# CloudEngineHub/dexrobot_isaac

Measured on AMD Instinct MI355X. Metric: env-steps/sec BlindGrasping num_envs=4096 per MI355X (random actions), higher is better.
Workload: dtype f32

## Files before the change

dexrobot_isaac_amd/csrc/dexsim_device.h:

```cpp
#pragma once
#include <hip/hip_runtime.h>

#include "../../include/dexsim.h"

#define DEXSIM_FIELDS(X)                                                                                    \
                                \
  X(float, q, 26) X(float, qd, 26) X(float, targets, 26)                                                    \
  X(float, box_pos, 3) X(float, box_quat, 4) X(float, box_lin, 3) X(float, box_ang, 3)                      \
  X(float, box_mass, 1) X(float, box_mu, 1)                                                                 \
                                                \
  X(float, site_pose, 77) X(float, hand_vel, 6) X(float, cforce, 51) X(float, cf5, 15)                      \
                                                    \
  X(float, jframe, 156) X(float, ufree, 32) X(float, fac_finv, 60)                                          \
  X(float, fac_g, 120) X(int, ncontact, 1) X(float, cgeom, DEXSIM_KMAX * 8) X(int, ccode, DEXSIM_KMAX)      \
  X(float, crow, DEXSIM_KMAX * 3 * 28) X(float, crowq, DEXSIM_KMAX * 3 * 28 + 4) X(float, clam, DEXSIM_KMAX * 3) X(float, chdr, DEXSIM_KMAX * 8) X(float, cstage, 6 * NP_STAGE * 9)                                         \
   \
  X(float, wlam, DEXSIM_NWKEY * 4) X(int, wgen, 1) X(int, csplit, 1)                                         \
        \
  X(float, active_prev_targets, 18) X(float, active_rule_targets, 18) X(float, prev_actions, 18)            \
  X(float, actions, 18) X(float, prev_dof_pos, 26)                                                          \
  X(float, contact_duration_steps, 5) X(float, prev_contact_binary, 5) X(int, episode_step, 1)              \
  X(int, success_duration_steps, 1) X(int, success_conditions_met, 1) X(int, current_stage, 1)              \
  X(int, just2, 1) X(int, just3, 1) X(float, time_in_stage, 1) X(float, stage_contact_duration, 1)          \
  X(float, initial_box_pos, 3)                                                                              \
  X(float, prev_finger_dof_vel, 20) X(float, prev_hand_vel, 3) X(float, prev_hand_ang_vel, 3)               \
  X(int, prev_contacts, 5)                                                                                  \
  X(int, episode_success, 1) X(int, episode_failure, 1) X(int, success_reason, DEXSIM_NUM_SUCC)             \
  X(int, failure_reason, DEXSIM_NUM_FAIL) X(int, crit_success, DEXSIM_NUM_SUCC)                             \
  X(int, crit_failure, DEXSIM_NUM_FAIL) X(int, term_success, 1) X(int, term_failure, 1)                     \
  X(int, term_timeout, 1)                                                                                   \
  X(float, obs_all, DEXSIM_OBS_ALL_DIM) X(float, rew_comp, DEXSIM_NUM_REWROWS) X(float, rew, 1)             \
  X(int, reset_flag, 1) X(int, reset_count, 1)

struct Arena {
#define X(type, name, rows) type* name;
  DEXSIM_FIELDS(X)
#undef X
};

#define FQ(field, quad) ((__attribute__((address_space(1))) f4*)(A.field) + ((size_t)(quad) * N + e))
#define JFRAME_FQ0 9
#define NP_STAGE 20
#define CSTAGE_CODE0 (6 * NP_STAGE * 8)

#define CROW_W 28

struct JC {
  float qoff[4], poff[3], axis[3], com[3], inertia[6];
  float mass, kp, kd, armature, lo, hi;
  float pad[7];
};
static_assert(sizeof(JC) == 128, "JC must be 128 bytes");

struct DevParams {
  DexSimConfig cfg;
  DexHandModel model;
  float h;
  float box_inv_I_k;
  float base_A[4][3], base_Oc[4][3], base_Q3z[4];
  unsigned obs_div_magic;
  int inertia_diag;
  float hand_reach;
  int obs_col_row[DEXSIM_OBS_ALL_DIM];
  JC jc[DEXSIM_NJ];
  Arena arena;
};

#define CNT_ANY_RESET 0
#define CNT_SUCC 1
#define CNT_FAIL 2
#define CNT_TERM_SUCCESS 8
#define CNT_TERM_FAILURE 9
#define CNT_TERM_TIMEOUT 10
#define CNT_NUM_RESETS 11
#define CNT_CONTACTS 16
#define CNT_HAND_CONTACTS 18
#define CNT_SPIN_TIMEOUT 20
#define CNT_PHYS_STEPS 13
#define CNT_CONSECUTIVE 14
#define CNT_RC_FIRST 15

typedef float f2 __attribute__((ext_vector_type(2)));
typedef float f4 __attribute__((ext_vector_type(4)));
__device__ __forceinline__ void st4_global(float* p, f4 v) { *(__attribute__((address_space(1))) f4*)p = v; }
__device__ __forceinline__ void st4_global(float* p, float a, float b, float c, float d) { f4 v; v.x = a; v.y = b; v.z = c; v.w = d; st4_global(p, v); }

struct V3 { float x, y, z; };
struct Q4 { float x, y, z, w; };
struct S6 { float xx, yy, zz, xy, xz, yz; };
struct M3 { float m[9]; };

#define DI __device__ __forceinline__

DI V3 v3(float x, float y, float z) { return {x, y, z}; }
DI V3 v3p(const float* p) { return {p[0], p[1], p[2]}; }
DI V3 operator+(V3 a, V3 b) { return {a.x + b.x, a.y + b.y, a.z + b.z}; }
DI V3 operator-(V3 a, V3 b) { return {a.x - b.x, a.y - b.y, a.z - b.z}; }
DI V3 operator*(float s, V3 a) { return {s * a.x, s * a.y, s * a.z}; }
DI V3& operator+=(V3& a, V3 b) { a.x += b.x; a.y += b.y; a.z += b.z; return a; }
DI V3& operator-=(V3& a, V3 b) { a.x -= b.x; a.y -= b.y; a.z -= b.z; return a; }
DI float dot(V3 a, V3 b) { return a.x * b.x + a.y * b.y + a.z * b.z; }
DI V3 cross(V3 a, V3 b) { return {a.y * b.z - a.z * b.y, a.z * b.x - a.x * b.z, a.x * b.y - a.y * b.x}; }
DI float norm(V3 a) { return sqrtf(dot(a, a)); }
DI float clampf(float x, float lo, float hi) { return x < lo ? lo : (x > hi ? hi : x); }

DI Q4 q4p(const float* p) { return {p[0], p[1], p[2], p[3]}; }
DI Q4 qmul(Q4 a, Q4 b) {
  return {a.w * b.x + a.x * b.w + a.y * b.z - a.z * b.y, a.w * b.y - a.x * b.z + a.y * b.w + a.z * b.x,
          a.w * b.z + a.x * b.y - a.y * b.x + a.z * b.w, a.w * b.w - a.x * b.x - a.y * b.y - a.z * b.z};
}
DI Q4 qconj(Q4 a) { return {-a.x, -a.y, -a.z, a.w}; }
DI M3 q2mat(Q4 q) {
  M3 R;
  float x = q.x, y = q.y, z = q.z, w = q.w;
  R.m[0] = 1 - 2 * (y * y + z * z); R.m[1] = 2 * (x * y - z * w); R.m[2] = 2 * (x * z + y * w);
  R.m[3] = 2 * (x * y + z * w); R.m[4] = 1 - 2 * (x * x + z * z); R.m[5] = 2 * (y * z - x * w);
  R.m[6] = 2 * (x * z - y * w); R.m[7] = 2 * (y * z + x * w); R.m[8] = 1 - 2 * (x * x + y * y);
  return R;
}
DI V3 mul(const M3& R, V3 v) {
  return {R.m[0] * v.x + R.m[1] * v.y + R.m[2] * v.z, R.m[3] * v.x + R.m[4] * v.y + R.m[5] * v.z,
          R.m[6] * v.x + R.m[7] * v.y + R.m[8] * v.z};
}
DI V3 mulT(const M3& R, V3 v) {
  return {R.m[0] * v.x + R.m[3] * v.y + R.m[6] * v.z, R.m[1] * v.x + R.m[4] * v.y + R.m[7] * v.z,
          R.m[2] * v.x + R.m[5] * v.y + R.m[8] * v.z};
}
DI V3 qrot_inv(Q4 q, V3 v) {
  V3 qv = {q.x, q.y, q.z};
  V3 c = cross(qv, v);
  float d = dot(qv, v), s = 2 * q.w * q.w - 1;
  return {v.x * s - 2 * q.w * c.x + 2 * qv.x * d, v.y * s - 2 * q.w * c.y + 2 * qv.y * d,
          v.z * s - 2 * q.w * c.z + 2 * qv.z * d};
}
DI V3 mul(S6 I, V3 v) {
  return {I.xx * v.x + I.xy * v.y + I.xz * v.z, I.xy * v.x + I.yy * v.y + I.yz * v.z,
          I.xz * v.x + I.yz * v.y + I.zz * v.z};
}
DI S6 operator+(S6 a, S6 b) { return {a.xx + b.xx, a.yy + b.yy, a.zz + b.zz, a.xy + b.xy, a.xz + b.xz, a.yz + b.yz}; }
DI S6 rotate_inertia(const M3& R, const float* s ) {
  float Il[9] = {s[0], s[3], s[4], s[3], s[1], s[5], s[4], s[5], s[2]};
  float T[9];
#pragma unroll
  for (int r = 0; r < 3; r++)
#pragma unroll
    for (int k = 0; k < 3; k++) T[3 * r + k] = R.m[3 * r] * Il[k] + R.m[3 * r + 1] * Il[3 + k] + R.m[3 * r + 2] * Il[6 + k];
  auto e = [&](int r, int k) { return T[3 * r] * R.m[3 * k] + T[3 * r + 1] * R.m[3 * k + 1] + T[3 * r + 2] * R.m[3 * k + 2]; };
  return {e(0, 0), e(1, 1), e(2, 2), e(0, 1), e(0, 2), e(1, 2)};
}
DI S6 rotate_inertia_diag(const M3& R, const float* s ) {
  const float a0 = s[0] * R.m[0], a3 = s[0] * R.m[3], a6 = s[0] * R.m[6];
  const float b1 = s[1] * R.m[1], b4 = s[1] * R.m[4], b7 = s[1] * R.m[7];
  const float c2 = s[2] * R.m[2], c5 = s[2] * R.m[5], c8 = s[2] * R.m[8];
  return {a0 * R.m[0] + b1 * R.m[1] + c2 * R.m[2], a3 * R.m[3] + b4 * R.m[4] + c5 * R.m[5], a6 * R.m[6] + b7 * R.m[7] + c8 * R.m[8],
          a0 * R.m[3] + b1 * R.m[4] + c2 * R.m[5], a0 * R.m[6] + b1 * R.m[7] + c2 * R.m[8], a3 * R.m[6] + b4 * R.m[7] + c5 * R.m[8]};
}
DI S6 pa(float m, V3 d) {
  float dd = dot(d, d);
  return {m * (dd - d.x * d.x), m * (dd - d.y * d.y), m * (dd - d.z * d.z), -m * d.x * d.y, -m * d.x * d.z, -m * d.y * d.z};
}

struct Comp { float m; V3 c; S6 I; };
DI void comp_add(Comp& a, const Comp& b) {
  float m = a.m + b.m;
  if (m <= 0.f) return;
  float inv = 1.f / m;
  V3 c = {(a.m * a.c.x + b.m * b.c.x) * inv, (a.m * a.c.y + b.m * b.c.y) * inv, (a.m * a.c.z + b.m * b.c.z) * inv};
  S6 I = a.I + b.I + pa(a.m * b.m * inv, a.c - b.c);
  a.m = m; a.c = c; a.I = I;
}

template <int n>
DI void spd_inverse(float* A) {
  float L[n * n];
#pragma unroll
  for (int i = 0; i < n; i++)
#pragma unroll
    for (int j = 0; j <= i; j++) {
      float s = A[i * n + j];
#pragma unroll
      for (int k = 0; k < j; k++) s -= L[i * n + k] * L[j * n + k];
      if (i == j) L[i * n + i] = sqrtf(fmaxf(s, 1e-20f));
      else L[i * n + j] = s / L[j * n + j];
    }
  float Li[n * n];
#pragma unroll
// ... 88 lines not shown
```

dexrobot_isaac_amd/csrc/dexsim_l2.hip.inc:

```

struct CouplingGroup { int n, dof[3]; float scale[3]; };
constexpr CouplingGroup kCoupling[18] = {
    {1, {0}, {1}}, {1, {1}, {1}}, {1, {2}, {1}}, {1, {3}, {1}}, {1, {4}, {1}}, {1, {5}, {1}},
    {1, {6}, {1}},
    {1, {7}, {1}},
    {2, {8, 9}, {1, 1}},
    {3, {10, 18, 22}, {1, 1, 2}},
    {1, {11}, {1}}, {2, {12, 13}, {1, 1}},
    {1, {15}, {1}}, {2, {16, 17}, {1, 1}},
    {1, {19}, {1}}, {2, {20, 21}, {1, 1}},
    {1, {23}, {1}}, {2, {24, 25}, {1, 1}},
};
constexpr int kHeldDof = 14;
constexpr int kActiveFingerDof[12] = {8, 7, 6, 10, 12, 11, 16, 15, 20, 19, 24, 23};

enum {
#define X(name, dim) O_##name, O_##name##_last = O_##name + (dim) - 1,
  DEXSIM_OBS_KEYS(X)
#undef X
  O_end
};
static_assert(O_end == DEXSIM_OBS_ALL_DIM, "DEXSIM_OBS_ALL_DIM is not the sum of the DEXSIM_OBS_KEYS dims");
static_assert(O_object_pos == DEXSIM_OBS_BASE_TASK_DIM, "DEXSIM_OBS_BASE_TASK_DIM is not the row of object_pos");

// ... 557 lines not shown
#pragma unroll 4
      for (int i = DEXSIM_OBS_BASE_TASK_DIM; i < DEXSIM_OBS_ALL_DIM; i++) OB(i) = 0.f;
    }
    post_logic_a(A, T, P, s_ob, in, mid, obs_only, N, NR);
  } else {
    if (wv == nw - 1)
      for (int i = lane; i < C.num_obs; i += 64) s_tab[i] = P->obs_col_row[i];
#pragma unroll 1
    for (int t = 0; t < POST_NTASK; t++)
      if (!((done_mask >> t) & 1) && (nw == 7 ? c_post_task_wave7[t] : c_post_task_wave[t] % nh) == wv - 1)
        post_task(t, A, P, cnt, s_ob, s_st, obs_only, N);
  }
  POST_STAMP();
  __syncthreads();
  const int r4 = lane >> 4, l16 = lane & 15;
  if (wv == 0) {
    if (!obs_only) post_logic_b(A, T, P, cnt, s_ob, s_st, in, mid, N, NR);
    if (fold_reset && e < NR && GPTR(A.reset_flag)[e] != 0) reset_phase0(A, T, P, N, NR, e);
  } else {
    const float* src = s_ob + (4 * l16) * OB_STRIDE + r4;
    if (!T.skip_obs_all)
    for (int g = wv - 1; g < DEXSIM_OBS_ALL_DIM / 4; g += nh) {
      const int row = 4 * g + r4;
      const f4 v = {src[4 * g], src[4 * g + OB_STRIDE], src[4 * g + 2 * OB_STRIDE], src[4 * g + 3 * OB_STRIDE]};
      st4_global(A.obs_all + (size_t)row * N + blockIdx.x * 64 + 4 * l16, v);
    }
    for (int g = wv - 1; g < 7; g += nh) {
      const int row = 4 * g + r4;
      if (row < 26) {
        const int ob = row < 6 ? O_base_dof_pos + row : O_all_finger_dof_pos + row - 6;
        const float* sq = s_ob + (4 * l16) * OB_STRIDE + ob;
        st4_global(A.prev_dof_pos + (size_t)row * N + blockIdx.x * 64 + 4 * l16, f4{sq[0], sq[OB_STRIDE], sq[2 * OB_STRIDE], sq[3 * OB_STRIDE]});
      }
    }
    const int O = C.num_obs;
    const int e0 = blockIdx.x * 64;
    const int nreal = min(64, NR - e0);
    const int total = nreal * O;
    const unsigned magic = P->obs_div_magic;
    float* dst = T.obs_buf + (size_t)e0 * O;
    float* dst2 = (T.sink_obs && !obs_only) ? T.sink_obs + (size_t)e0 * O : nullptr;
    for (int t4 = 4 * ((int)threadIdx.x - 64); t4 < total; t4 += 4 * ((int)blockDim.x - 64)) {
      float v[4];
#pragma unroll
      for (int j = 0; j < 4; j++) {
        const int idx = min(t4 + j, total - 1);
        const int el = (int)__umulhi((unsigned)idx, magic);
        const int c = idx - el * O;
        v[j] = s_ob[el * OB_STRIDE + s_tab[c]];
      }
      if (t4 + 3 < total) {
        st4_global(dst + t4, f4{v[0], v[1], v[2], v[3]});
        if (dst2) st4_global(dst2 + t4, f4{v[0], v[1], v[2], v[3]});
      } else {
        for (int j = 0; j < 4 && t4 + j < total; j++) { dst[t4 + j] = v[j]; if (dst2) dst2[t4 + j] = v[j]; }
      }
    }
  }
  POST_STAMP();
  __syncthreads();
  if (!obs_only) {
    for (int g = wv; g < (DEXSIM_NUM_REWROWS + 1 + 3) / 4; g += nw) {
      const int row = 4 * g + r4;
      if (row <= DEXSIM_NUM_REWROWS) {
        const float* sr = s_st + (ST_RC + row) * 64 + 4 * l16;
        const f4 v = {sr[0], sr[1], sr[2], sr[3]};
        float* dst = row < DEXSIM_NUM_REWROWS ? A.rew_comp + (size_t)row * N : A.rew;
        st4_global(dst + blockIdx.x * 64 + 4 * l16, v);
      }
    }
  }
  POST_STAMP();
  POST_STAMP();
#undef POST_STAMP
}

#define POST_LDS_BYTES ((64 * OB_STRIDE + 64 * ST_WORDS + DEXSIM_OBS_ALL_DIM) * sizeof(float))
__global__ __launch_bounds__(512) void k_post(Arena A, ApiPtrs T, const DevParams* __restrict__ P, int* __restrict__ cnt,
                                              int obs_only, int fold_reset, int N, int NR) {
  extern __shared__ float s_post[];
  post_block(P->arena, T, P, cnt, s_post, obs_only, fold_reset, N, NR, 0);
}

DI void finalize_stats(const ApiPtrs& T, const DevParams* __restrict__ P, int NR) {
  int* cnt = T.counters;
  float* st = T.stats;
  const DexSimConfig& C = P->cfg;
  auto mean = [&](int count) { return (float)((double)count / (double)NR); };
  st[DEXSIM_STAT_SUCC_MEAN] = mean(cnt[CNT_SUCC]);
  for (int i = 0; i < DEXSIM_NUM_FAIL; i++) st[DEXSIM_STAT_FAIL_MEAN + i] = mean(cnt[CNT_FAIL + i]);
  st[DEXSIM_STAT_SUCCESS_RATE] = mean(cnt[CNT_TERM_SUCCESS]);
  st[DEXSIM_STAT_FAILURE_RATE] = mean(cnt[CNT_TERM_FAILURE]);
  st[DEXSIM_STAT_TIMEOUT_RATE] = mean(cnt[CNT_TERM_TIMEOUT]);
  int cs = cnt[CNT_TERM_SUCCESS] > 0 ? cnt[CNT_CONSECUTIVE] + 1 : 0;
  if (cs > C.max_consecutive_successes) cs = C.max_consecutive_successes;
  cnt[CNT_CONSECUTIVE] = cs;
  st[DEXSIM_STAT_CONSECUTIVE_SUCCESSES] = (float)cs;
  st[DEXSIM_STAT_NUM_RESETS] = (float)cnt[CNT_NUM_RESETS];
  st[DEXSIM_STAT_PHYSICS_STEPS] = cnt[CNT_ANY_RESET] == T.stamp ? 2.f : 1.f;
  st[DEXSIM_STAT_MEAN_CONTACTS] = mean(cnt[CNT_CONTACTS + (T.stamp & 1)]);
  st[DEXSIM_STAT_MEAN_HAND_CONTACTS] = mean(cnt[CNT_HAND_CONTACTS + (T.stamp & 1)]);
  cnt[CNT_RC_FIRST] = 0;
  for (int i = CNT_SUCC; i <= CNT_NUM_RESETS; i++) cnt[i] = 0;
  if (T.sink_stats)
    for (int i = 0; i < DEXSIM_STAT_USED; i++) T.sink_stats[i] = st[i];
}

DI void reset_phase1(const Arena& A, int N, int e) {
#pragma unroll
  for (int f = 0; f < 5; f++) { FLD(contact_duration_steps, f) = 0.f; FLD(prev_contact_binary, f) = 0.f; }
#pragma unroll
  for (int i = 0; i < 26; i++) FLD(prev_dof_pos, i) = 0.f;
#pragma unroll
  for (int i = 0; i < 18; i++) FLD(prev_actions, i) = 0.f;
}

DI void reset_phase0(const Arena& A, const ApiPtrs& T, const DevParams* __restrict__ P, int N, int NR, int e) {
  const DexSimConfig& C = P->cfg;
  FLD(episode_success, 0) = 0; FLD(episode_failure, 0) = 0; FLD(success_reason, 0) = 0;
#pragma unroll
  for (int i = 0; i < DEXSIM_NUM_FAIL; i++) FLD(failure_reason, i) = 0;
  FLD(episode_step, 0) = 0;
  T.episode_step_count[e] = 0;
  T.episode_length[e] = 0;
  if (T.masks) {
#pragma unroll
    for (int i = 0; i < DEXSIM_NUM_SUCC + DEXSIM_NUM_FAIL; i++) T.masks[(size_t)(DEXSIM_MASK_SUCC_REASON + i) * NR + e] = 0;
  }
  float q[26];
#pragma unroll
  for (int i = 0; i < 26; i++) q[i] = 0.f;
  const int rc = FLD(reset_count, 0);
  if (C.task == DEXSIM_TASK_BLIND_GRASPING) {
    float u[32];
    if (T.reset_samples) {
#pragma unroll
      for (int i = 0; i < DEXSIM_NRESET_SAMPLES; i++) u[i] = T.reset_samples[(size_t)e * DEXSIM_NRESET_SAMPLES + i];
    } else {
#pragma unroll
      for (int b = 0; b < 8; b++) {
        uint32_t x[4];
        philox4x32(x, (uint32_t)e, (uint32_t)rc, (uint32_t)b, 0u, C.seed, 0x5eedu);
#pragma unroll
        for (int i = 0; i < 4; i++) u[4 * b + i] = u01(x[i]);
      }
    }
    const float x = (u[0] * 2.f - 1.f) * C.box_xy_range, y = (u[1] * 2.f - 1.f) * C.box_xy_range;
    const float yaw = (u[2] * 2.f - 1.f) * 3.14159265358979323846f;
    if (!C.box_fixed) {
      FLD(box_pos, 0) = x; FLD(box_pos, 1) = y; FLD(box_pos, 2) = C.box_z;
      FLD(initial_box_pos, 0) = x; FLD(initial_box_pos, 1) = y; FLD(initial_box_pos, 2) = C.box_z;
      FLD(box_quat, 0) = 0.f; FLD(box_quat, 1) = 0.f; FLD(box_quat, 2) = sinf(yaw / 2.f); FLD(box_quat, 3) = cosf(yaw / 2.f);
    }
#pragma unroll
    for (int i = 0; i < 3; i++) { FLD(box_lin, i) = 0.f; FLD(box_ang, i) = 0.f; }
    FLD(success_duration_steps, 0) = 0; FLD(success_conditions_met, 0) = 0;
    FLD(current_stage, 0) = 1; FLD(time_in_stage, 0) = 0.f; FLD(stage_contact_duration, 0) = 0.f;
    FLD(just2, 0) = 0; FLD(just3, 0) = 0;
#pragma unroll
    for (int i = 0; i < 3; i++) { q[i] = (u[3 + i] * 2.f - 1.f) * C.hand_translation_range; q[3 + i] = (u[6 + i] * 2.f - 1.f) * C.hand_rotation_range; }
#pragma unroll
    for (int i = 0; i < 20; i++) q[6 + i] = u[9 + i] * (i == 0 ? C.thumb_rotation_range : C.other_finger_range);
  }
  FLD(reset_count, 0) = rc + 1;
  FLD(wgen, 0) = DEXSIM_WGEN_NEXT(FLD(wgen, 0));
#pragma unroll
  for (int i = 0; i < 26; i++) {
    FLD(q, i) = q[i]; FLD(qd, i) = 0.f; FLD(targets, i) = q[i];
    if (T.full_dof_targets) T.full_dof_targets[(size_t)e * 26 + i] = q[i];
  }
#pragma unroll
  for (int c = 0; c < 18; c++) {
    const CouplingGroup& g = kCoupling[c];
    FLD(active_prev_targets, c) = q[g.dof[g.n - 1]] / g.scale[g.n - 1];
  }
}

__global__ __launch_bounds__(64) void k_reset(Arena A, ApiPtrs T, const DevParams* __restrict__ P, const int64_t* __restrict__ ids, int k,
                                              int mode, int phase, int N, int NR) {
  int e = blockIdx.x * 64 + threadIdx.x;
  if (mode == 3) {
    if (e >= NR || FLD(reset_flag, 0) == 0) return;
  } else {
    if (e >= k) return;
    if (mode == 1) e = (int)ids[e];
    if (e < 0 || e >= NR) return;
  }
  if (phase == 1) reset_phase1(A, N, e);
  else reset_phase0(A, T, P, N, NR, e);
}

__global__ void k_finalize(ApiPtrs T, const DevParams* __restrict__ P, int NR) {
  if (threadIdx.x != 0 || blockIdx.x != 0) return;
  finalize_stats(T, P, NR);
}

__global__ void k_begin_step(int* cnt, int stamp) {
  if (threadIdx.x == 0 && blockIdx.x == 0) begin_step_counters(cnt, stamp);
}

__global__ __launch_bounds__(64) void k_init(Arena A, ApiPtrs T, const DevParams* __restrict__ P, int N, int NR) {
  const int e = blockIdx.x * 64 + threadIdx.x;
  const DexSimConfig& C = P->cfg;
  FLD(box_quat, 3) = 1.f;
  FLD(box_pos, 2) = C.box_z;
  FLD(initial_box_pos, 2) = C.box_z;
  if (C.box_fixed) {
#pragma unroll
    for (int i = 0; i < 3; i++) { FLD(box_pos, i) = C.box_fixed_pos[i]; FLD(initial_box_pos, i) = C.box_fixed_pos[i]; }
  }
  float mass = C.box_mass > 0.f ? C.box_mass : 1.f, mu = C.box_friction;
  if (C.dr_enabled) {
    uint32_t x[4];
    philox4x32(x, (uint32_t)e, 0u, 0u, 0u, C.dr_seed, 0xd12au);
    mass = C.dr_mass_lo + u01(x[0]) * (C.dr_mass_hi - C.dr_mass_lo);
    mu = C.dr_mu_lo + u01(x[1]) * (C.dr_mu_hi - C.dr_mu_lo);
  }
  FLD(box_mass, 0) = mass; FLD(box_mu, 0) = mu;
  FLD(current_stage, 0) = 1;
  if (e == 0) {
    for (int i = 0; i < DEXSIM_STAT_WORDS; i++) { T.counters[i] = 0; T.stats[i] = 0.f; }
    T.counters[CNT_RC_FIRST] = 1;
  }
}

__global__ void k_ingest(Arena A, ApiPtrs T, const DevParams* __restrict__ P, const int64_t* __restrict__ ids, int k, int what,
                         int N, int NR) {
  const int i = blockIdx.x * blockDim.x + threadIdx.x;
  if (i >= k) return;
  const int e = (int)ids[i];
  if (e < 0 || e >= NR) return;
  if (what == 0) {
    for (int j = 0; j < 26; j++) { FLD(q, j) = T.dof_state[((size_t)e * 26 + j) * 2]; FLD(qd, j) = T.dof_state[((size_t)e * 26 + j) * 2 + 1]; }
  } else if (P->cfg.has_box) {
    const float* b = T.root_state + ((size_t)e * 2 + 1) * 13;
    for (int j = 0; j < 3; j++) { FLD(box_pos, j) = b[j]; FLD(box_lin, j) = b[7 + j]; FLD(box_ang, j) = b[10 + j]; }
    for (int j = 0; j < 4; j++) FLD(box_quat, j) = b[3 + j];
  }
}
```

dexrobot_isaac_amd/csrc/dexsim_physics.hip.inc:

```

#define GPTR(p) ((__attribute__((address_space(1))) __typeof__(*(p))*)(p))
#define FLD(f, r) GPTR(A.f)[(size_t)(r) * N + e]
#define ROWADDR(w, lane) ((((w) >> 2) * 64 + (lane)) * 4 + ((w) & 3))

DI int wave_role(int w) { return w == 2 ? 5 : ((w >= 3 && w <= 5) ? w - 1 : w); }
#ifndef SPEC_SPLIT_NUM
#define SPEC_SPLIT_NUM 12
#endif

#define CODE_TYPE(c) ((c) & 3)
#define CODE_CAP(c) (((c) >> 2) & 31)
#define CODE_SAMPLE(c) (((c) >> 7) & 7)
#define CODE_FINGER(c) ((((c) >> 16) & 7) - 1)
#define CODE_LEVEL(c) (((c) >> 19) & 3)
#define CODE_FSLOT(c) (((c) >> 21) & 31)
DI int code_info(const DexHandModel& M, int cap) {
  const int jp = M.cap_parent[cap];
  return ((jp >= 6 ? ((jp - 6) >> 2) + 1 : 0) << 16) | ((jp >= 6 ? (jp - 6) & 3 : 0) << 19) | (M.cap_fslot[cap] << 21);
}
#define CODE_HKEY(c) (CODE_TYPE(c) == 3 ? 88 + ((CODE_FINGER(c) * 4 + CODE_LEVEL(c)) * 2 + (CODE_SAMPLE(c) & 1)) \
                                         : (CODE_CAP(c) * 2 + CODE_TYPE(c)) * 2 + (CODE_SAMPLE(c) & 1))
#define SPLIT_NB(s) ((s) & 15)
#define SPLIT_NX(s) (((s) >> 4) & 15)
#define SPLIT_NF(s, f) (((s) >> (8 + 4 * (f))) & 15)
// ... 347 lines not shown
    }
  }
  return -1;
}
static_assert(FS_LDS_BYTES == 160 * 1024, "the sub-step kernels own the CU's whole LDS: one workgroup per CU");
static_assert(lds_map_conflict() < 0, "LDS map: a region leaves the LDS or shares a word with a region live in a common phase "
                                      "(the note shows 1000 x the first word of one + the first word of the other)");
static_assert(DL_CAPS(0, 5) == DL_HANDOFF, "the per-finger hand-off is DL_HANDOFF words");
#define SOLVE_LDS_WORDS(kstage) (60 + DEXSIM_KMAX * 3 + DEXSIM_KMAX * 4 + (kstage) * 3 * CROW_W)
static_assert((DL_SPLIT + 1) * 64 * sizeof(float) <= FS_LDS_BYTES, "k_dynamics' LDS does not fit into the CU's");
static_assert(SOLVE_LDS_WORDS(4) * 64 * sizeof(float) <= FS_LDS_BYTES, "k_solve's LDS does not fit into the CU's");

struct FingerIn { float ql[4], qdl[4], tg[4]; };
DI void finger_load(const Arena& A, int f, int N, int e, FingerIn& in) {
#pragma unroll
  for (int l = 0; l < 4; l++) { const int j = 6 + 4 * f + l; in.ql[l] = FLD(q, j); in.qdl[l] = FLD(qd, j); in.tg[l] = FLD(targets, j); }
}

DI bool finger_dynamics(const Arena& A, const DevParams* __restrict__ P, const BaseChain& B, const FingerIn& in, float* sh, const int dlb,
                        float* s_uf, int lane, int f, int N, int e, int tok_seq = 0, bool sphere_clear = false,
                        V3 bpos = V3{0, 0, 0}, const M3& Rb = M3{{1, 0, 0, 0, 1, 0, 0, 0, 1}}, float* Gk = nullptr) {
  const DexHandModel& M = P->model;
  const float h = P->h;
  const int j0 = 6 + 4 * f;
  Q4 qf = B.q5; V3 of = B.o5; V3 wf = B.w5, alf = B.al5, aof = B.ao5;
  V3 a[4], o[4], cl[4], fl[4], nl[4];
  S6 Iw[4];
  float ql[4], qdl[4], tg[4];
  bool clr = true;
  if (tok_seq > 0 && sphere_clear && lane == 0) sh[(FS_FLAG + f) * 64] = __int_as_float((tok_seq << 1) | 1);
#pragma unroll
  for (int l = 0; l < 4; l++) {
    const int j = j0 + l;
    ql[l] = in.ql[l]; qdl[l] = in.qdl[l]; tg[l] = in.tg[l];
    M3 Rp = q2mat(qf);
    V3 on = of + mul(Rp, v3p(P->jc[j].poff));
    Q4 qz = qmul(qf, q4p(P->jc[j].qoff));
    V3 ax = v3p(P->jc[j].axis);
    float s, c;
    sincos_joint(0.5f * ql[l], &s, &c);
    Q4 qn = qmul(qz, Q4{ax.x * s, ax.y * s, ax.z * s, c});
    M3 R = q2mat(qn);
    V3 aw = mul(R, ax);
    V3 r = on - of;
    V3 aoj = aof + cross(alf, r) + cross(wf, cross(wf, r));
    V3 cw = cross(wf, aw);
    alf += qdl[l] * cw; wf += qdl[l] * aw; aof = aoj;
    cl[l] = on + mul(R, v3p(P->jc[j].com));
    Iw[l] = (tok_seq > 0 && P->inertia_diag) ? rotate_inertia_diag(R, P->jc[j].inertia) : rotate_inertia(R, P->jc[j].inertia);
    V3 rc = cl[l] - on;
    V3 ac = aof + cross(alf, rc) + cross(wf, cross(wf, rc));
    fl[l] = P->jc[j].mass * ac;
    nl[l] = mul(Iw[l], alf) + cross(wf, mul(Iw[l], wf)) + cross(rc, fl[l]);
    if (l >= 1 && !(tok_seq > 0 && sphere_clear)) {
      const int cap = 3 + 3 * f + (l - 1);
      const V3 c0 = on + mul(R, v3p(M.cap_p0[cap])), c1 = on + mul(R, v3p(M.cap_p1[cap]));
      sh_put3(sh, lane, DL_CAPS(dlb, f) + 6 * (l - 1), c0);
      sh_put3(sh, lane, DL_CAPS(dlb, f) + 6 * (l - 1) + 3, c1);
      if (tok_seq > 0) clr = clr && capsule_clear(c0, c1, M.cap_r[cap], P->cfg, bpos, Rb);
    }
    a[l] = aw; o[l] = on; qf = qn; of = on;
  }
  bool fclear = false;
  if (tok_seq > 0) {
    fclear = sphere_clear || __all(clr);
    if (!sphere_clear && lane == 0) sh[(FS_FLAG + f) * 64] = __int_as_float((tok_seq << 1) | (fclear ? 1 : 0));
  }
  if (!fclear) {
    const float w24[24] = {a[0].x, a[0].y, a[0].z, o[0].x, o[0].y, o[0].z, a[1].x, a[1].y, a[1].z, o[1].x, o[1].y, o[1].z,
                           a[2].x, a[2].y, a[2].z, o[2].x, o[2].y, o[2].z, a[3].x, a[3].y, a[3].z, o[3].x, o[3].y, o[3].z};
#pragma unroll
    for (int qd = 0; qd < 6; qd++) *FQ(jframe, JFRAME_FQ0 + 6 * f + qd) = f4{w24[4 * qd], w24[4 * qd + 1], w24[4 * qd + 2], w24[4 * qd + 3]};
  }
  float bias[4];
#pragma unroll
  for (int l = 3; l >= 0; l--) {
    bias[l] = dot(a[l], nl[l]);
    if (l > 0) { fl[l - 1] += fl[l]; nl[l - 1] += nl[l] + cross(o[l] - o[l - 1], fl[l]); }
  }
  sh_put3(sh, lane, DL_WRENCH(dlb, f), fl[0]);
  sh_put3(sh, lane, DL_WRENCH(dlb, f) + 3, nl[0] + cross(o[0] - B.o5, fl[0]));
  float Fm[16], Cm[24];
  Comp cc;
#pragma unroll
  for (int l = 3; l >= 0; l--) {
    Comp b; b.m = P->jc[j0 + l].mass; b.c = cl[l]; b.I = Iw[l];
    if (l == 3) cc = b; else { comp_add(b, cc); cc = b; }
    V3 Pm = cc.m * cross(a[l], cc.c - o[l]);
    V3 Lm = mul(cc.I, a[l]);
#pragma unroll
    for (int k = 0; k <= l; k++) {
      float v = dot(a[k], Lm + cross(cc.c - o[k], Pm));
      Fm[l * 4 + k] = v; Fm[k * 4 + l] = v;
    }
#pragma unroll
    for (int i = 0; i < 6; i++)
      Cm[i * 4 + l] = i < 3 ? dot(B.ab[i], Pm) : dot(B.ab[i], Lm + cross(cc.c - B.ob[i], Pm));
  }
  comp_put(sh, lane, DL_COMP(dlb, f), cc, B.o5);
  if (tok_seq > 0) {
    asm volatile("" ::: "memory");
    if (lane == 0) __hip_atomic_fetch_add((int*)(sh + FS_COMPCNT * 64), 1, __ATOMIC_RELAXED, __HIP_MEMORY_SCOPE_WORKGROUP);
  }
  float tau[4];
#pragma unroll
  for (int l = 0; l < 4; l++) {
    const int j = j0 + l;
    const float kp = P->jc[j].kp, kdh = P->jc[j].kd + h * kp;
    Fm[l * 4 + l] += P->jc[j].armature + h * kdh;
    tau[l] = kp * (tg[l] - ql[l]) - kdh * qdl[l] - bias[l];
  }
  spd_inverse<4>(Fm);
  float G[24];
  f2 G2[12];
#pragma unroll
  for (int l = 0; l < 4; l++)
#pragma unroll
    for (int ip = 0; ip < 3; ip++) {
      f2 s2 = {0.f, 0.f};
#pragma unroll
      for (int k = 0; k < 4; k++) s2 = f2{Cm[(2 * ip) * 4 + k], Cm[(2 * ip + 1) * 4 + k]} * Fm[l * 4 + k] + s2;
      G2[l * 3 + ip] = s2;
      G[l * 6 + 2 * ip] = s2.x; G[l * 6 + 2 * ip + 1] = s2.y;
    }
  if (!(tok_seq > 0 && sphere_clear && Gk)) {
#pragma unroll
    for (int qd = 0; qd < 6; qd++) *FQ(fac_g, 6 * f + qd) = f4{G[4 * qd], G[4 * qd + 1], G[4 * qd + 2], G[4 * qd + 3]};
  }
  if (Gk) {
#pragma unroll
    for (int i = 0; i < 24; i++) Gk[i] = G[i];
  }
#pragma unroll
  for (int i = 0; i < 6; i++)
#pragma unroll
    for (int kp = 0; kp <= i / 2; kp++) {
      f2 s2 = {0.f, 0.f};
#pragma unroll
      for (int l = 0; l < 4; l++) s2 = G2[l * 3 + kp] * Cm[i * 4 + l] + s2;
      SH(DL_SSUB(dlb, f) + i * (i + 1) / 2 + 2 * kp) = s2.x;
      if (2 * kp + 1 <= i) SH(DL_SSUB(dlb, f) + i * (i + 1) / 2 + 2 * kp + 1) = s2.y;
    }
  if (!fclear) {
    *FQ(fac_finv, 3 * f) = f4{Fm[0], Fm[4], Fm[5], Fm[8]};
    *FQ(fac_finv, 3 * f + 1) = f4{Fm[9], Fm[10], Fm[12], Fm[13]};
    *FQ(fac_finv, 3 * f + 2) = f4{Fm[14], Fm[15], 0.f, 0.f};
  }
#pragma unroll
  for (int ip = 0; ip < 3; ip++) {
    f2 s2 = {0.f, 0.f};
#pragma unroll
    for (int l = 0; l < 4; l++) s2 = G2[l * 3 + ip] * tau[l] + s2;
    SH(DL_GSUM(dlb, f) + 2 * ip) = s2.x; SH(DL_GSUM(dlb, f) + 2 * ip + 1) = s2.y;
  }
#pragma unroll
  for (int l = 0; l < 4; l++) {
    float s = qdl[l];
#pragma unroll
    for (int i = 0; i < 6; i++) s += G[l * 6 + i] * B.qdb[i];
    float acc = 0.f;
#pragma unroll
    for (int k = 0; k < 4; k++) acc += Fm[l * 4 + k] * tau[k];
    const float uf = s + h * acc;
    if (s_uf) s_uf[(4 * f + l) * 64 + lane] = uf;
    else FLD(ufree, j0 + l) = uf;
  }
  return fclear;
}

#define SCHUR_SPLIT_BIT (1 << 30)
#ifdef DEXSIM_DEBUG_SPIN
#define SPIN_GUARD_INIT() int spin_polls_ = 0
#define SPIN_GUARD(cntp, site, seq) if (++spin_polls_ > (DEXSIM_DEBUG_SPIN)) { if (cntp) GPTR(cntp)[CNT_SPIN_TIMEOUT] = ((site) << 24) | (seq); break; }
#else
#define SPIN_GUARD_INIT() do {} while (0)
#define SPIN_GUARD(cntp, site, seq) do {} while (0)
#endif
DI Comp schur_comp(const float* sh, const int dlb, int lane, V3 o5) {
  float M = SH(DL_PALM);
  V3 sd = M * sh_get3(sh, lane, DL_PALM + 1);
  S6 J = {SH(DL_PALM + 4), SH(DL_PALM + 5), SH(DL_PALM + 6), SH(DL_PALM + 7), SH(DL_PALM + 8), SH(DL_PALM + 9)};
#pragma unroll
  for (int f = 0; f < 5; f++) {
    const float mf = SH(DL_COMP(dlb, f));
    M += mf;
    sd += mf * sh_get3(sh, lane, DL_COMP(dlb, f) + 1);
    J = J + S6{SH(DL_COMP(dlb, f) + 4), SH(DL_COMP(dlb, f) + 5), SH(DL_COMP(dlb, f) + 6), SH(DL_COMP(dlb, f) + 7), SH(DL_COMP(dlb, f) + 8), SH(DL_COMP(dlb, f) + 9)};
  }
  const float inv = M > 0.f ? 1.f / M : 0.f;
  const V3 d = inv * sd;
  const S6 sh_back = pa(M, d);
  Comp c;
  c.m = M; c.c = o5 + d;
  c.I = {J.xx - sh_back.xx, J.yy - sh_back.yy, J.zz - sh_back.zz, J.xy - sh_back.xy, J.xz - sh_back.xz, J.yz - sh_back.yz};
  return c;
}
template <int i, int k0 = 0, int k1 = i>
DI void schur_row(float* sh, const int dlb, int lane) {
  float r[k1 - k0 + 1];
#pragma unroll
  for (int k = k0; k <= k1; k++) {
    const float v = SH(FS_SPRE + i * (i + 1) / 2 + k);
    float ss = 0.f;
#pragma unroll
    for (int f = 0; f < 5; f++) ss += SH(DL_SSUB(dlb, f) + i * (i + 1) / 2 + k);
    r[k - k0] = v - ss;
  }
#pragma unroll
  for (int k = k0; k <= k1; k++) SH(DL_SCHUR_S + i * (i + 1) / 2 + k) = r[k - k0];
}
DI void schur_precompute(float* sh, const int dlb, int lane, const BaseChain& B, int seq, int* dbg_cnt) {
  {
    SPIN_GUARD_INIT();
    while (*(volatile int*)(sh + FS_COMPCNT * 64) < 5 * seq) { __builtin_amdgcn_s_sleep(2); SPIN_GUARD(dbg_cnt, 4, seq); }
  }
  asm volatile("" ::: "memory");
  const Comp comp5 = schur_comp(sh, dlb, lane, B.o5);
  int idx = 0;
#pragma unroll
  for (int i = 0; i < 6; i++) {
    V3 Pm, Lm;
    if (i < 3) { Pm = comp5.m * B.ab[i]; Lm = {0, 0, 0}; }
    else { Pm = comp5.m * cross(B.ab[i], comp5.c - B.ob[i]); Lm = mul(comp5.I, B.ab[i]); }
#pragma unroll
    for (int k = 0; k <= i; k++) {
      SH(FS_SPRE + idx) = k < 3 ? dot(B.ab[k], Pm) : dot(B.ab[k], Lm + cross(comp5.c - B.ob[k], Pm));
      idx++;
    }
  }
  V3 ff = sh_get3(sh, lane, DL_PALM_WRENCH), nn = sh_get3(sh, lane, DL_PALM_WRENCH + 3);
#pragma unroll
  for (int f = 0; f < 5; f++) {
    ff += sh_get3(sh, lane, DL_WRENCH(dlb, f));
    nn += sh_get3(sh, lane, DL_WRENCH(dlb, f) + 3);
  }
  SH(FS_SPRE_BIAS + 5) = dot(B.ab[5], nn);
#pragma unroll
  for (int j = 4; j >= 0; j--) {
    nn += cross(B.ob[j + 1] - B.ob[j], ff);
    SH(FS_SPRE_BIAS + j) = j < 3 ? dot(B.ab[j], ff) : dot(B.ab[j], nn);
  }
}
DI void schur_helper(float* sh, const int dlb, int job, int lane) {
  if (job == 1) {
    float gsum[6] = {0, 0, 0, 0, 0, 0};
#pragma unroll
    for (int f = 0; f < 5; f++)
#pragma unroll
      for (int i = 0; i < 6; i++) gsum[i] += SH(DL_GSUM(dlb, f) + i);
#pragma unroll
    for (int i = 0; i < 6; i++) SH(DL_SCHUR_GSUM + i) = gsum[i];
    schur_row<0>(sh, dlb, lane); schur_row<1>(sh, dlb, lane); schur_row<2>(sh, dlb, lane);
  } else if (job == 0) {
    schur_row<3>(sh, dlb, lane); schur_row<5, 4, 5>(sh, dlb, lane);
  } else schur_row<4>(sh, dlb, lane);
}

DI void schur_base(const Arena& A, const DevParams* __restrict__ P, const BaseChain& B, float* sh, const int dlb, float* uB_out,
                   int lane, int N, int e, int tgt_lds = -1, bool solve_only = false, int split_seq = 0,
                   unsigned long long dbg_t0 = 0, int dbg_row = 0, int* dbg_cnt = nullptr) {
#if defined(DEXSIM_PROFILE_PHASES) && defined(DBG_SCHUR)
#define SCHUR_STAMP(i) do { if (lane == 0) A.crow[(size_t)(dbg_row + (i)) * N + e] = __int_as_float((int)(__builtin_amdgcn_s_memtime() - dbg_t0)); } while (0)
#else
#define SCHUR_STAMP(i) do {} while (0)
#endif
  const float h = P->h;
  SCHUR_STAMP(0);
  Comp comp5;
  V3 f5 = sh_get3(sh, lane, DL_PALM_WRENCH), n5 = sh_get3(sh, lane, DL_PALM_WRENCH + 3);
  float Ssub[21], gsum[6] = {0, 0, 0, 0, 0, 0};
#pragma unroll
  for (int i = 0; i < 21; i++) Ssub[i] = 0.f;
  if (split_seq == 0) comp5 = schur_comp(sh, dlb, lane, B.o5);
  if (split_seq == 0) {
#pragma unroll
    for (int f = 0; f < 5; f++) {
      f5 += sh_get3(sh, lane, DL_WRENCH(dlb, f));
      n5 += sh_get3(sh, lane, DL_WRENCH(dlb, f) + 3);
#pragma unroll
      for (int i = 0; i < 21; i++) Ssub[i] += SH(DL_SSUB(dlb, f) + i);
#pragma unroll
      for (int i = 0; i < 6; i++) gsum[i] += SH(DL_GSUM(dlb, f) + i);
    }
  }
  SCHUR_STAMP(1);
  float S[36];
  if (split_seq > 0) schur_row<5, 0, 3>(sh, dlb, lane);
  else {
    int idx = 0;
#pragma unroll
    for (int i = 0; i < 6; i++) {
      V3 Pm, Lm;
      if (i < 3) { Pm = comp5.m * B.ab[i]; Lm = {0, 0, 0}; }
      else { Pm = comp5.m * cross(B.ab[i], comp5.c - B.ob[i]); Lm = mul(comp5.I, B.ab[i]); }
#pragma unroll
      for (int k = 0; k <= i; k++) {
        float v = k < 3 ? dot(B.ab[k], Pm) : dot(B.ab[k], Lm + cross(comp5.c - B.ob[k], Pm));
        v -= Ssub[idx++];
        S[i * 6 + k] = v; S[k * 6 + i] = v;
      }
    }
  }
  SCHUR_STAMP(2);
  float tauB[6];
  float bias[6];
  if (split_seq > 0) {
    const int want = (split_seq << 1) | 1 | SCHUR_SPLIT_BIT;
#pragma unroll 1
    for (int w = 1; w <= 3; w++) {
      SPIN_GUARD_INIT();
      while (__float_as_int(*(volatile float*)(sh + (FS_FLAG + w) * 64)) != want) { __builtin_amdgcn_s_sleep(1); SPIN_GUARD(dbg_cnt, 1, split_seq); }
    }
    asm volatile("" ::: "memory");
    SCHUR_STAMP(3);
    {
      int idx = 0;
#pragma unroll
      for (int i = 0; i < 6; i++)
#pragma unroll
        for (int k = 0; k <= i; k++) {
          const float v = SH(DL_SCHUR_S + idx); idx++;
          S[i * 6 + k] = v; S[k * 6 + i] = v;
        }
    }
#pragma unroll
    for (int i = 0; i < 6; i++) { bias[i] = SH(FS_SPRE_BIAS + i); gsum[i] = SH(DL_SCHUR_GSUM + i); }
  } else {
    V3 nn = n5, ff = f5;
    bias[5] = dot(B.ab[5], nn);
#pragma unroll
    for (int j = 4; j >= 0; j--) {
      nn += cross(B.ob[j + 1] - B.ob[j], ff);
      bias[j] = j < 3 ? dot(B.ab[j], ff) : dot(B.ab[j], nn);
    }
// ... 1696 lines not shown
      t1[0] = uB[4]; t1[1] = uB[5];
    } else if (wv == 6) {
      float* t1 = (float*)TQ(1);
      t1[2] = SH(FS_BOXV); t1[3] = SH(FS_BOXV + 1);
      *TQ(2) = f4{SH(FS_BOXV + 2), SH(FS_BOXV + 3), SH(FS_BOXV + 4), SH(FS_BOXV + 5)};
    }
    if (wv < 5) *TQ(3 + wv) = f4{s_uf[(4 * wv) * 64 + lane], s_uf[(4 * wv + 1) * 64 + lane], s_uf[(4 * wv + 2) * 64 + lane], s_uf[(4 * wv + 3) * 64 + lane]};
  }
#pragma unroll
    for (int i = 0; i < 24; i++) Gkeep[i] = 0.f;
    unsigned long long pr_t3 = 0;
    if (T.probe && wv == 0) pr_t3 = __builtin_amdgcn_s_memtime();
#ifdef DEXSIM_PROFILE_PHASES
    general_contact_phases(P, N, wv, lane, e, t_start, stamp_base, T.probe);
    stamp_i += 2;
#else
    general_contact_phases(P, N, wv, lane, e, 0ull, 0, T.probe);
#endif
    if (T.probe && wv == 0 && lane == 0) {
      atomicAdd(T.probe + blockIdx.x * 4, (unsigned)(__builtin_amdgcn_s_memtime() - pr_t3));
      atomicAdd(T.probe + blockIdx.x * 4 + 2, 1u);
    }
  } else if (early) {
    PHASE_STAMP(); PHASE_STAMP();
  }

  if (last && gp) {
    if (wv < 5) forces_partial(A, P, s_hdr, s_lam, sh + (FS_FORCE + wv * DEXSIM_NFSLOT * 3) * 64, nc, wv, lane, N, e);
    __syncthreads();
  }
#pragma unroll
  for (int i = 0; i < 6; i++) uB[i] = SH(FS_UB + i);
  const bool store_q = LAST || !carry_out || C.joint_limit_rows != 0;
  if (wv < 5) {
    const int f = wv;
    float G[24];
    if (sphere) {
#pragma unroll
      for (int i = 0; i < 24; i++) G[i] = Gkeep[i];
    } else {
#pragma unroll
      for (int qd = 0; qd < 6; qd++) { const f4 g4 = *FQ(fac_g, 6 * f + qd); G[4 * qd] = g4.x; G[4 * qd + 1] = g4.y; G[4 * qd + 2] = g4.z; G[4 * qd + 3] = g4.w; }
    }
#pragma unroll
    for (int l = 0; l < 4; l++) {
      float v = s_uf[(4 * f + l) * 64 + lane];
#pragma unroll
      for (int i = 0; i < 6; i++) v -= G[l * 6 + i] * uB[i];
      float qn = 0.f, vn = 0.f;
      integrate_joint(A, P, h, 6 + 4 * f + l, fin.ql[l], v, N, e, &qn, &vn, store_q);
      if (carry_out) { carry.ql[l] = qn; carry.qdl[l] = vn; carry.tg[l] = fin.tg[l]; }
    }
  } else if (wv == 5) {
#pragma unroll
    for (int i = 0; i < 6; i++) {
      float qn = 0.f, vn = 0.f;
      integrate_joint(A, P, h, i, B.qb[i], uB[i], N, e, &qn, &vn, store_q);
      if (carry_out) { SH(FS_CARRY_Q + i) = qn; SH(FS_CARRY_QD + i) = vn; }
    }
  } else {
    if (has_box) {
      float vb[3], wb[3];
#pragma unroll
      for (int i = 0; i < 3; i++) { vb[i] = SH(FS_BOXV + i); wb[i] = SH(FS_BOXV + 3 + i); }
      if (carry_out) { SH(FS_CARRY_BP) = fmaf(h, vb[0], bpos.x); SH(FS_CARRY_BP + 1) = fmaf(h, vb[1], bpos.y); SH(FS_CARRY_BP + 2) = fmaf(h, vb[2], bpos.z); }
      if (!C.box_fixed) integrate_box(A, h, vb, wb, N, e);
    }
  }
  if (last && wv < 5 && gp) forces_reduce(A, ccnt, s_hdr, sh + FS_FORCE * 64, nc, lane, N, e, NR, wv, 5);
  if (last && wv == 5 && gp) contact_stats(ccnt, s_hdr, nc, lane, e, NR);
  PHASE_STAMP();
  }
  if (LAST) {
    __syncthreads();
    publish_body(A, T, P, 0, N, NR, 6);
    if (post_pre && wv == 6) post_pre_tasks(A, P, cnt, sh, N);
    PHASE_STAMP();
  }
#undef PHASE_STAMP
#undef PH2_STAMP
}

DI void reset_phase1(const Arena& A, int N, int e);
DI void finalize_stats(const ApiPtrs& T, const DevParams* __restrict__ P, int NR);
DI void post_block(const Arena& A, const ApiPtrs& T, const DevParams* __restrict__ P, int* __restrict__ cnt, float* s_ob,
                   int obs_only, int fold_reset, int N, int NR, int done_mask);
DI void actions_block(const Arena& A, const ApiPtrs& T, const DevParams* __restrict__ P, const float* __restrict__ act,
                      int zero_targets, int N, int NR);

enum {
  TAIL_RESET = 1,
  TAIL_POST = 2,
  TAIL_NOT_FINAL = 4,
};

template <bool GATED>
DI unsigned long long physics_prologue(const ApiPtrs& T, float* sh) {
  unsigned long long pr_k0 = 0;
  if (T.probe && threadIdx.x == 0) pr_k0 = __builtin_amdgcn_s_memtime();
  if (threadIdx.x < 6) sh[(FS_FLAG + threadIdx.x) * 64] = 0.f;
  if (threadIdx.x == 6) sh[FS_COMPCNT * 64] = 0.f;
  return pr_k0;
}
template <bool GATED>
DI void physics_epilogue(const ApiPtrs& T, const DevParams* __restrict__ P, int tail, unsigned long long pr_k0, int NR) {
  if (GATED && (tail & TAIL_RESET) && blockIdx.x == 0 && threadIdx.x == 0) finalize_stats(T, P, NR);
  if (!GATED && T.probe && threadIdx.x == 0) atomicAdd(T.probe + blockIdx.x * 4 + 1, (unsigned)(__builtin_amdgcn_s_memtime() - pr_k0));
}

template <bool GATED>
__global__ __launch_bounds__(448) void k_physics4(Arena A, ApiPtrs T, const DevParams* __restrict__ P, int* __restrict__ cnt,
                                                  const float* __restrict__ act, int tail, int N, int NR) {
  extern __shared__ float sh[];
  const unsigned long long pr_k0 = physics_prologue<GATED>(T, sh);
  if (!GATED && act) actions_block(P->arena, T, P, act, 0, N, NR);
  __syncthreads();
  if (!GATED || cnt[CNT_ANY_RESET] == T.stamp) {
    SubstepCarry K;
    substep_body<false>(P->arena, T, P, cnt, N, NR, sh, 1, 64, false, true, K, false, true);
    __syncthreads();
    substep_body<false>(P->arena, T, P, cnt, N, NR, sh, 2, 128, false, true, K, true, true);
    __syncthreads();
    substep_body<false>(P->arena, T, P, cnt, N, NR, sh, 3, 192, false, true, K, true, true);
    __syncthreads();
    substep_body<true>(P->arena, T, P, cnt, N, NR, sh, 4, 256, !GATED && (tail & TAIL_POST), !GATED && !(tail & TAIL_NOT_FINAL), K, true, false);
    if (!GATED && (tail & TAIL_POST)) {
      __syncthreads();
      post_block(P->arena, T, P, cnt, sh, 0, 1, N, NR, POST_PRE_MASK);
    }
    if (GATED && (tail & TAIL_RESET)) {
      const int e = blockIdx.x * 64 + (threadIdx.x & 63);
      if (threadIdx.x < 64 && e < NR && A.reset_flag[e] != 0) reset_phase1(A, N, e);
    }
  }
  physics_epilogue<GATED>(T, P, tail, pr_k0, NR);
}

template <bool GATED>
__global__ __launch_bounds__(448) void k_physics1(Arena A, ApiPtrs T, const DevParams* __restrict__ P, int* __restrict__ cnt,
                                                  const float* __restrict__ act, int tail, int N, int NR) {
  extern __shared__ float sh[];
  const unsigned long long pr_k0 = physics_prologue<GATED>(T, sh);
  if (!GATED && act) actions_block(P->arena, T, P, act, 0, N, NR);
  __syncthreads();
  if (!GATED || cnt[CNT_ANY_RESET] == T.stamp) {
    SubstepCarry K;
    substep_body<true>(P->arena, T, P, cnt, N, NR, sh, 1, 0, !GATED && (tail & TAIL_POST), !GATED && !(tail & TAIL_NOT_FINAL), K, false, false);
    if (!GATED && (tail & TAIL_POST)) {
      __syncthreads();
      post_block(P->arena, T, P, cnt, sh, 0, 1, N, NR, POST_PRE_MASK);
    }
    if (GATED && (tail & TAIL_RESET)) {
      const int e = blockIdx.x * 64 + (threadIdx.x & 63);
      if (threadIdx.x < 64 && e < NR && A.reset_flag[e] != 0) reset_phase1(A, N, e);
    }
  }
  physics_epilogue<GATED>(T, P, tail, pr_k0, NR);
}
```

Measured before the change: 65.80 million.

## Pack composite-inertia and Schur sums into float2 ops; parallelize stats finalize across a wavefront

Rewrites part of the composite-inertia Fm/Cm computation and the Schur row and gsum reductions to use packed float2 arithmetic, aiming to let the compiler emit packed FP32 instructions and cut VALU issue count. Separately, finalize_stats goes from a single thread doing serial loads and stores to 64 lanes, each handling one stat slot, with a waitcnt before the counter clears. The packed paths add register pressure and asm register pins. The lane-parallel finalize relies on the ordering of reads before clears within one wavefront.

```diff
diff --git a/dexrobot_isaac_amd/csrc/dexsim_device.h b/dexrobot_isaac_amd/csrc/dexsim_device.h
--- a/dexrobot_isaac_amd/csrc/dexsim_device.h
+++ b/dexrobot_isaac_amd/csrc/dexsim_device.h
@@ -102,6 +102,14 @@
 DI float dot(V3 a, V3 b) { return a.x * b.x + a.y * b.y + a.z * b.z; }
 DI V3 cross(V3 a, V3 b) { return {a.y * b.z - a.z * b.y, a.z * b.x - a.x * b.z, a.x * b.y - a.y * b.x}; }
 DI float norm(V3 a) { return sqrtf(dot(a, a)); }
+struct V32 { f2 x, y, z; };
+DI V32 pk(V3 a, V3 b) { return {f2{a.x, b.x}, f2{a.y, b.y}, f2{a.z, b.z}}; }
+DI V3 vreg(V3 a) { asm("" : "+v"(a.x), "+v"(a.y), "+v"(a.z)); return a; }
+DI V32 bc(V3 a) { return {f2{a.x, a.x}, f2{a.y, a.y}, f2{a.z, a.z}}; }
+DI V32 operator+(V32 a, V32 b) { return {a.x + b.x, a.y + b.y, a.z + b.z}; }
+DI V32 operator-(V32 a, V32 b) { return {a.x - b.x, a.y - b.y, a.z - b.z}; }
+DI f2 dot(V32 a, V32 b) { return a.x * b.x + a.y * b.y + a.z * b.z; }
+DI V32 cross(V32 a, V32 b) { return {a.y * b.z - a.z * b.y, a.z * b.x - a.x * b.z, a.x * b.y - a.y * b.x}; }
 DI float clampf(float x, float lo, float hi) { return x < lo ? lo : (x > hi ? hi : x); }
 
 DI Q4 q4p(const float* p) { return {p[0], p[1], p[2], p[3]}; }
diff --git a/dexrobot_isaac_amd/csrc/dexsim_l2.hip.inc b/dexrobot_isaac_amd/csrc/dexsim_l2.hip.inc
--- a/dexrobot_isaac_amd/csrc/dexsim_l2.hip.inc
+++ b/dexrobot_isaac_amd/csrc/dexsim_l2.hip.inc
@@ -663,28 +663,37 @@
   post_block(P->arena, T, P, cnt, s_post, obs_only, fold_reset, N, NR, 0);
 }
 
-DI void finalize_stats(const ApiPtrs& T, const DevParams* __restrict__ P, int NR) {
+DI void finalize_stats(const ApiPtrs& T, const DevParams* __restrict__ P, int NR, int lane) {
   int* cnt = T.counters;
   float* st = T.stats;
   const DexSimConfig& C = P->cfg;
-  auto mean = [&](int count) { return (float)((double)count / (double)NR); };
-  st[DEXSIM_STAT_SUCC_MEAN] = mean(cnt[CNT_SUCC]);
-  for (int i = 0; i < DEXSIM_NUM_FAIL; i++) st[DEXSIM_STAT_FAIL_MEAN + i] = mean(cnt[CNT_FAIL + i]);
-  st[DEXSIM_STAT_SUCCESS_RATE] = mean(cnt[CNT_TERM_SUCCESS]);
-  st[DEXSIM_STAT_FAILURE_RATE] = mean(cnt[CNT_TERM_FAILURE]);
-  st[DEXSIM_STAT_TIMEOUT_RATE] = mean(cnt[CNT_TERM_TIMEOUT]);
-  int cs = cnt[CNT_TERM_SUCCESS] > 0 ? cnt[CNT_CONSECUTIVE] + 1 : 0;
-  if (cs > C.max_consecutive_successes) cs = C.max_consecutive_successes;
-  cnt[CNT_CONSECUTIVE] = cs;
-  st[DEXSIM_STAT_CONSECUTIVE_SUCCESSES] = (float)cs;
-  st[DEXSIM_STAT_NUM_RESETS] = (float)cnt[CNT_NUM_RESETS];
-  st[DEXSIM_STAT_PHYSICS_STEPS] = cnt[CNT_ANY_RESET] == T.stamp ? 2.f : 1.f;
-  st[DEXSIM_STAT_MEAN_CONTACTS] = mean(cnt[CNT_CONTACTS + (T.stamp & 1)]);
-  st[DEXSIM_STAT_MEAN_HAND_CONTACTS] = mean(cnt[CNT_HAND_CONTACTS + (T.stamp & 1)]);
-  cnt[CNT_RC_FIRST] = 0;
-  for (int i = CNT_SUCC; i <= CNT_NUM_RESETS; i++) cnt[i] = 0;
-  if (T.sink_stats)
-    for (int i = 0; i < DEXSIM_STAT_USED; i++) T.sink_stats[i] = st[i];
+  const int par = T.stamp & 1;
+  int w = -1;
+  if (lane >= DEXSIM_STAT_SUCC_MEAN && lane < DEXSIM_STAT_SUCC_MEAN + DEXSIM_NUM_SUCC) w = CNT_SUCC + lane - DEXSIM_STAT_SUCC_MEAN;
+  else if (lane >= DEXSIM_STAT_FAIL_MEAN && lane < DEXSIM_STAT_FAIL_MEAN + DEXSIM_NUM_FAIL) w = CNT_FAIL + lane - DEXSIM_STAT_FAIL_MEAN;
+  else if (lane >= DEXSIM_STAT_SUCCESS_RATE && lane <= DEXSIM_STAT_TIMEOUT_RATE) w = CNT_TERM_SUCCESS + lane - DEXSIM_STAT_SUCCESS_RATE;
+  else if (lane == DEXSIM_STAT_CONSECUTIVE_SUCCESSES) w = CNT_TERM_SUCCESS;
+  else if (lane == DEXSIM_STAT_NUM_RESETS) w = CNT_NUM_RESETS;
+  else if (lane == DEXSIM_STAT_PHYSICS_STEPS) w = CNT_ANY_RESET;
+  else if (lane == DEXSIM_STAT_MEAN_CONTACTS) w = CNT_CONTACTS + par;
+  else if (lane == DEXSIM_STAT_MEAN_HAND_CONTACTS) w = CNT_HAND_CONTACTS + par;
+  const int count = w >= 0 ? cnt[w] : 0;
+  float v = (float)((double)count / (double)NR);
+  if (lane == DEXSIM_STAT_NUM_RESETS) v = (float)count;
+  if (lane == DEXSIM_STAT_PHYSICS_STEPS) v = count == T.stamp ? 2.f : 1.f;
+  if (lane == DEXSIM_STAT_CONSECUTIVE_SUCCESSES) {
+    int cs = count > 0 ? cnt[CNT_CONSECUTIVE] + 1 : 0;
+    if (cs > C.max_consecutive_successes) cs = C.max_consecutive_successes;
+    cnt[CNT_CONSECUTIVE] = cs;
+    v = (float)cs;
+  }
+  if (lane < DEXSIM_STAT_USED) {
+    if (w >= 0) st[lane] = v; else v = st[lane];
+    if (T.sink_stats) T.sink_stats[lane] = v;
+  }
+  asm volatile("s_waitcnt vmcnt(0)" ::: "memory");
+  if (lane == 0) cnt[CNT_RC_FIRST] = 0;
+  if (lane >= CNT_SUCC && lane <= CNT_NUM_RESETS) cnt[lane] = 0;
 }
 
 DI void reset_phase1(const Arena& A, int N, int e) {
@@ -772,8 +781,8 @@
 }
 
 __global__ void k_finalize(ApiPtrs T, const DevParams* __restrict__ P, int NR) {
-  if (threadIdx.x != 0 || blockIdx.x != 0) return;
-  finalize_stats(T, P, NR);
+  if (threadIdx.x >= 64 || blockIdx.x != 0) return;
+  finalize_stats(T, P, NR, threadIdx.x);
 }
 
 __global__ void k_begin_step(int* cnt, int stamp) {
diff --git a/dexrobot_isaac_amd/csrc/dexsim_physics.hip.inc b/dexrobot_isaac_amd/csrc/dexsim_physics.hip.inc
--- a/dexrobot_isaac_amd/csrc/dexsim_physics.hip.inc
+++ b/dexrobot_isaac_amd/csrc/dexsim_physics.hip.inc
@@ -453,20 +453,29 @@
   sh_put3(sh, lane, DL_WRENCH(dlb, f) + 3, nl[0] + cross(o[0] - B.o5, fl[0]));
   float Fm[16], Cm[24];
   Comp cc;
+  const V32 ab45 = pk(vreg(B.ab[4]), vreg(B.ab[5])), ob45 = pk(vreg(B.ob[4]), vreg(B.ob[5]));
+  const V32 a01 = pk(a[0], a[1]), o01 = pk(o[0], o[1]);
 #pragma unroll
   for (int l = 3; l >= 0; l--) {
     Comp b; b.m = P->jc[j0 + l].mass; b.c = cl[l]; b.I = Iw[l];
     if (l == 3) cc = b; else { comp_add(b, cc); cc = b; }
     V3 Pm = cc.m * cross(a[l], cc.c - o[l]);
     V3 Lm = mul(cc.I, a[l]);
-#pragma unroll
-    for (int k = 0; k <= l; k++) {
+    const V32 Pm2 = bc(Pm), Lm2 = bc(Lm), c2 = bc(cc.c);
+#pragma unroll
+    for (int k = (l >= 2 ? 2 : 0); k <= l; k++) {
       float v = dot(a[k], Lm + cross(cc.c - o[k], Pm));
       Fm[l * 4 + k] = v; Fm[k * 4 + l] = v;
     }
-#pragma unroll
-    for (int i = 0; i < 6; i++)
+    if (l >= 2) {
+      const f2 v = dot(a01, Lm2 + cross(c2 - o01, Pm2));
+      Fm[l * 4] = v.x; Fm[l] = v.x; Fm[l * 4 + 1] = v.y; Fm[4 + l] = v.y;
+    }
+#pragma unroll
+    for (int i = 0; i < 4; i++)
       Cm[i * 4 + l] = i < 3 ? dot(B.ab[i], Pm) : dot(B.ab[i], Lm + cross(cc.c - B.ob[i], Pm));
+    const f2 c45 = dot(ab45, Lm2 + cross(c2 - ob45, Pm2));
+    Cm[4 * 4 + l] = c45.x; Cm[5 * 4 + l] = c45.y;
   }
   comp_put(sh, lane, DL_COMP(dlb, f), cc, B.o5);
   if (tok_seq > 0) {
@@ -568,17 +577,25 @@
 }
 template <int i, int k0 = 0, int k1 = i>
 DI void schur_row(float* sh, const int dlb, int lane) {
-  float r[k1 - k0 + 1];
-#pragma unroll
-  for (int k = k0; k <= k1; k++) {
-    const float v = SH(FS_SPRE + i * (i + 1) / 2 + k);
+  constexpr int n = k1 - k0 + 1, w0 = i * (i + 1) / 2 + k0;
+  f2 r2[n / 2 + 1];
+#pragma unroll
+  for (int k = 0; k + 1 < n; k += 2) {
+    const f2 v = {SH(FS_SPRE + w0 + k), SH(FS_SPRE + w0 + k + 1)};
+    f2 ss = {0.f, 0.f};
+#pragma unroll
+    for (int f = 0; f < 5; f++) ss += f2{SH(DL_SSUB(dlb, f) + w0 + k), SH(DL_SSUB(dlb, f) + w0 + k + 1)};
+    r2[k / 2] = v - ss;
+  }
+  if (n & 1) {
+    const float v = SH(FS_SPRE + w0 + n - 1);
     float ss = 0.f;
 #pragma unroll
-    for (int f = 0; f < 5; f++) ss += SH(DL_SSUB(dlb, f) + i * (i + 1) / 2 + k);
-    r[k - k0] = v - ss;
-  }
-#pragma unroll
-  for (int k = k0; k <= k1; k++) SH(DL_SCHUR_S + i * (i + 1) / 2 + k) = r[k - k0];
+    for (int f = 0; f < 5; f++) ss += SH(DL_SSUB(dlb, f) + w0 + n - 1);
+    r2[n / 2].x = v - ss;
+  }
+#pragma unroll
+  for (int k = 0; k < n; k++) SH(DL_SCHUR_S + w0 + k) = (k & 1) ? r2[k / 2].y : r2[k / 2].x;
 }
 DI void schur_precompute(float* sh, const int dlb, int lane, const BaseChain& B, int seq, int* dbg_cnt) {
   {
@@ -614,13 +631,13 @@
 }
 DI void schur_helper(float* sh, const int dlb, int job, int lane) {
   if (job == 1) {
-    float gsum[6] = {0, 0, 0, 0, 0, 0};
+    f2 gsum[3] = {{0.f, 0.f}, {0.f, 0.f}, {0.f, 0.f}};
 #pragma unroll
     for (int f = 0; f < 5; f++)
 #pragma unroll
-      for (int i = 0; i < 6; i++) gsum[i] += SH(DL_GSUM(dlb, f) + i);
-#pragma unroll
-    for (int i = 0; i < 6; i++) SH(DL_SCHUR_GSUM + i) = gsum[i];
+      for (int ip = 0; ip < 3; ip++) gsum[ip] += f2{SH(DL_GSUM(dlb, f) + 2 * ip), SH(DL_GSUM(dlb, f) + 2 * ip + 1)};
+#pragma unroll
+    for (int ip = 0; ip < 3; ip++) { SH(DL_SCHUR_GSUM + 2 * ip) = gsum[ip].x; SH(DL_SCHUR_GSUM + 2 * ip + 1) = gsum[ip].y; }
     schur_row<0>(sh, dlb, lane); schur_row<1>(sh, dlb, lane); schur_row<2>(sh, dlb, lane);
   } else if (job == 0) {
     schur_row<3>(sh, dlb, lane); schur_row<5, 4, 5>(sh, dlb, lane);
@@ -2483,7 +2500,7 @@
 }
 
 DI void reset_phase1(const Arena& A, int N, int e);
-DI void finalize_stats(const ApiPtrs& T, const DevParams* __restrict__ P, int NR);
+DI void finalize_stats(const ApiPtrs& T, const DevParams* __restrict__ P, int NR, int lane);
 DI void post_block(const Arena& A, const ApiPtrs& T, const DevParams* __restrict__ P, int* __restrict__ cnt, float* s_ob,
                    int obs_only, int fold_reset, int N, int NR, int done_mask);
 DI void actions_block(const Arena& A, const ApiPtrs& T, const DevParams* __restrict__ P, const float* __restrict__ act,
@@ -2505,7 +2522,7 @@
 }
 template <bool GATED>
 DI void physics_epilogue(const ApiPtrs& T, const DevParams* __restrict__ P, int tail, unsigned long long pr_k0, int NR) {
-  if (GATED && (tail & TAIL_RESET) && blockIdx.x == 0 && threadIdx.x == 0) finalize_stats(T, P, NR);
+  if (GATED && (tail & TAIL_RESET) && blockIdx.x == 0 && threadIdx.x < 64) finalize_stats(T, P, NR, threadIdx.x);
   if (!GATED && T.probe && threadIdx.x == 0) atomicAdd(T.probe + blockIdx.x * 4 + 1, (unsigned)(__builtin_amdgcn_s_memtime() - pr_k0));
 }
 
```

Result: no change. 66.24 million, median of 6 (+0.7%).
